# zdebruine/MMVAE

Hardware: AMD Instinct MI355X
Metric: cells/sec per MMVAE train step (higher is better)
Workload: dtype f32; 1 GPU; c2: 2-modality MMVAE train step, 20000 genes each, latent 128, K=1, batch 512/GPU, adversarial=False; global_batch=512, parallelism=dp1, exchange=none

## Files before the change

### include/mmvae_hip.h

```cpp
#ifndef MMVAE_HIP_H
#define MMVAE_HIP_H

#include <stddef.h>
#include <stdint.h>

#ifdef __cplusplus
extern "C" {
#endif

typedef void* mmvae_stream_t;

#define MMVAE_OK 0
#define MMVAE_ERR_ARG 1
#define MMVAE_ERR_LAUNCH 2
#define MMVAE_ERR_WORKSPACE 3

#define MMVAE_ABI_VERSION 16
int mmvae_abi_version(void);
const char* mmvae_build_arch(void);

#define MMVAE_GEMM_NT 0
#define MMVAE_GEMM_NN 1
#define MMVAE_GEMM_TN 2

// ... 197 lines not shown
typedef struct {
    const float* A;
    const float* B;
    float* C;
    const float* bias;
    int64_t lda, ldb, ldc;
    int32_t layout, M, N, K;
    float alpha;
    uint32_t flags;
    int32_t first_block;
    int32_t n_blocks;
} mmvae_gemm_job;
int mmvae_gemm_batch_job_ok(const mmvae_gemm_job* job);
int mmvae_gemm_batch_prepare(int n_jobs, mmvae_gemm_job* jobs, int* total_blocks);
int mmvae_gemm_batch_f32(int n_jobs, const mmvae_gemm_job* jobs_dev, int total_blocks, mmvae_stream_t stream);

int mmvae_csr_to_dense_f32(int B, int G, int64_t nnz, const int64_t* crow_indices, const int64_t* col_indices,
                           const float* values, float* out, int64_t ldo, mmvae_stream_t stream);
int mmvae_csr_to_dense_i32_f32(int B, int G, int64_t nnz, const int32_t* crow_indices, const int32_t* col_indices,
                               const float* values, float* out, int64_t ldo, mmvae_stream_t stream);

int mmvae_csr_gather_rows_i64(int B, int64_t n_src_rows, int64_t src_nnz, const int64_t* src_crow, const int64_t* src_col,
                              const float* src_val, const int64_t* rows, const int64_t* out_crow, int64_t out_nnz,
                              int64_t* out_col, float* out_val, mmvae_stream_t stream);
int mmvae_csr_gather_rows_i32(int B, int64_t n_src_rows, int64_t src_nnz, const int32_t* src_crow, const int32_t* src_col,
                              const float* src_val, const int64_t* rows, const int32_t* out_crow, int64_t out_nnz,
                              int32_t* out_col, float* out_val, mmvae_stream_t stream);
int mmvae_csr_gather_rows_dense_i64(int B, int G, int64_t n_src_rows, int64_t src_nnz, const int64_t* src_crow,
                                    const int64_t* src_col, const float* src_val, const int64_t* rows, float* out,
                                    int64_t ldo, mmvae_stream_t stream);
// ... 132 lines not shown
```

### mmvae_amd/_lib.py

```python
from __future__ import annotations

import ctypes as C
import os
from typing import Optional

_HERE = os.path.dirname(os.path.abspath(__file__))
LIB_PATH = os.path.join(_HERE, "csrc", "libmmvae_hip.so")
if os.environ.get("MMVAE_LIB"):
    LIB_PATH = os.environ["MMVAE_LIB"]

OK, ERR_ARG, ERR_LAUNCH, ERR_WORKSPACE = 0, 1, 2, 3
_ERR_NAMES = {1: "MMVAE_ERR_ARG", 2: "MMVAE_ERR_LAUNCH", 3: "MMVAE_ERR_WORKSPACE"}

GEMM_NT, GEMM_NN, GEMM_TN = 0, 1, 2
GEMM_RELU, GEMM_ACCUMULATE, GEMM_RAW_SLABS, GEMM_OPERAND_SLACK = 1, 2, 4, 8
GEMM_PRECISION_F32, GEMM_PRECISION_BF16X3 = 0, 1
ADAM_STATE_FLOATS = 8
ADAM_HYPER_FLOATS = 4
PREPARE_NORM, PREPARE_ADVANCE = 1, 2

_p = C.c_void_p
_i = C.c_int
_l = C.c_int64
_f = C.c_float
# ... 16 lines not shown


class Planes(C.Structure):
    _fields_ = [("p", _p), ("ld", _l), ("plane_stride", _l)]


class ReconArgs(C.Structure):
    _fields_ = [("rows", C.c_int32), ("x_rows", C.c_int32), ("G", C.c_int32), ("H", C.c_int32), ("flags", C.c_uint32),
                ("reserved", C.c_uint32), ("h", _p), ("W", _p), ("bias", _p), ("x", _p), ("ldh", _l), ("ldw", _l),
                ("ldx", _l), ("xhat", _p), ("dP", _p), ("se_part", _p), ("col_part", _p), ("ldxhat", _l), ("lddp", _l),
                ("h_planes", Planes), ("W_planes", Planes), ("dP_planes", Planes)]


class SplitJob(C.Structure):
    _fields_ = [("rows", C.c_int32), ("cols", C.c_int32), ("src", _p), ("ld_src", _l), ("planes", Planes)]


RECON_H_KPAD = 1


PROTOTYPES = {
    "mmvae_abi_version": (_i, []),
    "mmvae_build_arch": (C.c_char_p, []),
    "mmvae_gemm_set_precision": (_i, [_i]),
    "mmvae_gemm_set_workgroup_cap": (_i, [_i]),
    "mmvae_adam_set_workgroups": (_i, [_i]),
    "mmvae_adam_get_workgroups": (_i, []),
    "mmvae_gemm_set_x3w": (_i, [_i]),
    "mmvae_gemm_get_x3w": (_i, []),
    "mmvae_gemm_get_precision": (_i, []),
# ... 68 lines not shown
    "mmvae_csr_gather_rows_i64": (_i, [_i, _l, _l, _p, _p, _p, _p, _p, _l, _p, _p, _p]),
    "mmvae_csr_gather_rows_i32": (_i, [_i, _l, _l, _p, _p, _p, _p, _p, _l, _p, _p, _p]),
    "mmvae_csr_gather_rows_dense_i64": (_i, [_i, _i, _l, _l, _p, _p, _p, _p, _p, _l, _p]),
    "mmvae_csr_gather_rows_dense_i32": (_i, [_i, _i, _l, _l, _p, _p, _p, _p, _p, _l, _p]),
    "mmvae_csr_spmm_wt_i32_f32": (_i, [_i, _i, _i, _l, _p, _p, _p, _p, _l, _p, _p, _l, _p]),
    "mmvae_cond_linear_fwd": (_i, [_i, _i, _i, _p, _l, _p, _p, _p, _p, _p, _p, _l, _p]),
    "mmvae_cond_linear_bwd_dx": (_i, [_i, _i, _i, _p, _l, _p, _p, _p, _p, _p, _l, _i, _p]),
    "mmvae_cond_linear_bwd_dw": (_i, [_i, _p, _p, _p, _p, _i, _i, _p, _l, _p, _l, _p, _p, _p, _i, _p, _p, _p, _p, _p]),
    "mmvae_cond_linear_fwd_multi": (_i, [_i, _i, _i, _i, _p, _l, _l, _p, _p, _p, _p, _p, _l, _p, _l, _l, _p]),
    "mmvae_cond_linear_bwd_dx_multi": (_i, [_i, _i, _i, _i, _p, _l, _l, _p, _p, _p, _l, _p, _l, _i, _p]),
    "mmvae_cond_linear_bwd_dw_multi": (_i, [_i, _i, _p, _p, _p, _p, _l, _i, _i, _p, _l, _l, _p, _l, _l, _p, _p, _p, _i, _p,
                                            _p, _p, _p, _l, _p]),
    "mmvae_gemm_batch_job_ok": (_i, [_p]),
    "mmvae_gemm_batch_prepare": (_i, [_i, _p, C.POINTER(_i)]),
    "mmvae_gemm_batch_f32": (_i, [_i, _p, _i, _p]),
    "mmvae_adv_pass_plan": (_i, [_p, _i, C.POINTER(_i), C.POINTER(_z), C.POINTER(_l), C.POINTER(_i)]),
    "mmvae_adv_pass_f32": (_i, [_i, _p, _i, _i, _i, _i, _z, _p]),
    "mmvae_adv_dw_prepare": (_i, [_i, _p, C.POINTER(_i), C.POINTER(_i)]),
    "mmvae_adv_dw_f32": (_i, [_i, _p, _i, _i, _p, _p, _p, _i, _p, _i, _p]),
    "mmvae_adam_step_multi_hp": (_i, [_i, _p, _l, _p]),
    "mmvae_ell_from_dense_f32": (_i, [_i, _i, _p, _l, _i, _p, _p, _p, _p]),
    "mmvae_dw_sparse_ell_f32": (_i, [_i, _i, _i, _p, _l, _p, _p, _p, _i, _p, _l, _p]),
    "mmvae_col_pearson_workspace_bytes": (_z, [_i, _i]),
    "mmvae_col_pearson_f32": (_i, [_i, _i, _p, _l, _p, _l, _p, _p, _z, _p]),
}


class SumJob(C.Structure):
    _fields_ = [("src", C.c_void_p), ("dst", C.c_void_p), ("part_stride", C.c_int64), ("ld_src", C.c_int64),
                ("ld_dst", C.c_int64), ("n_parts", C.c_int32), ("rows", C.c_int32), ("cols", C.c_int32),
# ... 84 lines not shown
```

### mmvae_amd/csrc/gemm_dev.h

```cpp
#pragma once
#include "common.h"
#include <type_traits>

namespace mmvae_detail {
struct GemmArgs {
    const float* A;
    const float* B;
    float* C;
    const float* bias;
    int64_t lda, ldb, ldc;
    int M, N, K;
    int mt, nt;
    int ktiles;
    int ktiles_per_split;
    int64_t slab_stride;
    float alpha;
    unsigned flags;
    int aligned;
    int x3_vec;
    const float* x;
    float* xhat;
    float* dP;
    float* se_part;
    int64_t ldx, ldxhat, lddp;
    int x_rows;
    int se_tiles;
    int c_vec;
    int nwork;
    float* sq_part;
    float* col_part;
    const unsigned short* Ap;
    const unsigned short* Bp;
    int64_t ldap, ldbp, a_pstride, b_pstride;
    unsigned short* dPp;
    int64_t lddpp, dp_pstride;
};
bool x3w_planes_combo(int layout, bool a_pl, bool b_pl);
int launch_x3w_planes(int layout, int tile_id, bool a_pl, bool b_pl, int epi, const GemmArgs& g, int nwork, int slots,
                      hipStream_t s);

}

namespace {

#ifndef MMVAE_GEMM_BK0
#define MMVAE_GEMM_BK0 32
#endif
#ifndef MMVAE_X3_PERSISTENT
#define MMVAE_X3_PERSISTENT 0
#endif
#ifndef MMVAE_X3_STAMPS
#define MMVAE_X3_STAMPS 0
#endif
#ifndef MMVAE_SLAB_STORE_NT
#define MMVAE_SLAB_STORE_NT 0
#endif
#ifndef MMVAE_GEMM_PRELOAD
#define MMVAE_GEMM_PRELOAD 0
#endif

constexpr int NT = 256;

enum { FORM_KC = 0, FORM_RC = 1 };
enum { EPI_STD = 0, EPI_RECON = 1 };

template <int FORM, int R, int BK>
struct Tile {
    static constexpr int KC_LD = BK + 4;
    static constexpr int LDS_FLOATS = (FORM == FORM_KC) ? R * KC_LD : BK * R;
    static constexpr int NVEC = R * BK / 4;
    static constexpr int VECS = (NVEC + NT - 1) / NT;
    static constexpr bool EXACT = (NVEC % NT) == 0;
    static constexpr int C4 = (FORM == FORM_KC) ? BK / 4 : R / 4;
};

using mmvae_detail::GemmArgs;


template <int FORM, int R, int BK, bool VEC, int NV>
// ... 1571 lines not shown
```

### mmvae_amd/csrc/gemm_f32.hip

```cpp
#include "gemm_dev.h"

namespace {

template <int AFORM, int BFORM, int BM, int BN, int BK>
struct F32Lds {
    static constexpr int A_FLOATS = Tile<AFORM, BM, BK>::LDS_FLOATS, B_FLOATS = Tile<BFORM, BN, BK>::LDS_FLOATS;
    static constexpr int FLOATS = 2 * A_FLOATS + 2 * B_FLOATS;
};

template <int AFORM, int BFORM, int BM, int BN, int BK, int WGM, int WGN, bool VEC, int EPI>
__device__ __forceinline__ void gemm_f32_item(const GemmArgs& g, int L, float* lds) {
    static_assert(WGM * WGN == 4, "4 wavefronts per workgroup");
    constexpr int WTM = BM / WGM, WTN = BN / WGN;
    constexpr int TM = WTM / 32, TN = WTN / 32;
    static_assert(TM * 32 == WTM && TN * 32 == WTN && BK % 8 == 0, "tile shape");
    using TA = Tile<AFORM, BM, BK>;
    using TB = Tile<BFORM, BN, BK>;
    constexpr int A_FLOATS = TA::LDS_FLOATS, B_FLOATS = TB::LDS_FLOATS;
    constexpr int KK = BK / 8;
    float* As = lds;
    float* Bs = lds + 2 * A_FLOATS;

    const int tid = threadIdx.x;
    const int lane = tid & 63;
// ... 70 lines not shown
#pragma unroll
                    for (int i = 0; i < TM; ++i)
#pragma unroll
                        for (int n = 0; n < TN; ++n)
                            acc[i][n] = __builtin_amdgcn_mfma_f32_32x32x2f32(fa[i][j], fb[n][j], acc[i][n], 0, 0, 0);
            }
#endif
            if (more) {
                store_tile<AFORM, BM, BK>(As + (cur ^ 1) * A_FLOATS, ra, va, tid);
                store_tile<BFORM, BN, BK>(Bs + (cur ^ 1) * B_FLOATS, rb, vb, tid);
            }
            __syncthreads();
        }
    }

    gemm_epilogue<BM, BN, WGM, WGN, EPI>(acc, g, bm, bn, z, lds);
}

template <int AFORM, int BFORM, int BM, int BN, int BK, int WGM, int WGN, bool VEC, int EPI>
__global__ __launch_bounds__(NT) void gemm_f32_kernel(const GemmArgs g) {
    __shared__ __attribute__((aligned(16))) float lds[F32Lds<AFORM, BFORM, BM, BN, BK>::FLOATS];
    gemm_f32_item<AFORM, BFORM, BM, BN, BK, WGM, WGN, VEC, EPI>(g, xcd_remap(blockIdx.x, gridDim.x), lds);
}

__global__ __launch_bounds__(NT) void gemm_f32_batch_kernel(const mmvae_gemm_job* __restrict__ jobs, int n_jobs) {
    constexpr int LDS_FLOATS = F32Lds<FORM_KC, FORM_KC, 64, 64, 32>::FLOATS;
    static_assert(LDS_FLOATS >= F32Lds<FORM_KC, FORM_RC, 64, 64, 32>::FLOATS &&
                      LDS_FLOATS >= F32Lds<FORM_RC, FORM_RC, 64, 64, 32>::FLOATS, "LDS size");
    __shared__ __attribute__((aligned(16))) float lds[LDS_FLOATS];
    const int L = xcd_remap(blockIdx.x, gridDim.x);
    int j = 0;
// ... 1046 lines not shown
    *total_blocks = (int)first;
    return MMVAE_OK;
}

extern "C" int mmvae_gemm_batch_f32(int n_jobs, const mmvae_gemm_job* jobs_dev, int total_blocks,
                                    mmvae_stream_t stream) {
    if (n_jobs <= 0 || !jobs_dev || total_blocks <= 0) return MMVAE_ERR_ARG;
    if (x3s_enabled())
        MMVAE_LAUNCH(gemm_x3s_batch_kernel, dim3(total_blocks), dim3(NT), 0, (hipStream_t)stream, jobs_dev, n_jobs);
    else
        MMVAE_LAUNCH(gemm_f32_batch_kernel, dim3(total_blocks), dim3(NT), 0, (hipStream_t)stream, jobs_dev, n_jobs);
    MMVAE_LAUNCH_CHECK();
    return MMVAE_OK;
}

extern "C" int mmvae_recon_tiles(int G) {
    if (G <= 0) return 0;
    return ceil_div_i(G, g_precision == MMVAE_GEMM_PRECISION_BF16X3 ? 128 : 160);
}

#if MMVAE_X3_STAMPS
extern "C" int mmvae_debug_x3_stamps(long long* out32) {
    return hipMemcpyFromSymbol(out32, HIP_SYMBOL(g_x3_stamps), sizeof(long long) * 32) == hipSuccess ? 0 : 1;
}
extern "C" int mmvae_debug_x3_trace(long long* out, int n_blocks) {
    return hipMemcpyFromSymbol(out, HIP_SYMBOL(g_x3_trace), sizeof(long long) * 4 * n_blocks) == hipSuccess ? 0 : 1;
}
#endif

extern "C" int mmvae_gemm_set_precision(int mode) {
// ... 111 lines not shown
```

### mmvae_amd/engine.py

```python
from __future__ import annotations

import os
from dataclasses import dataclass
from typing import Dict, List, Optional

import torch

from . import _lib, dist as mdist, rng
from .constants import REGISTRY_KEYS as RK
from .engine_adv import PlanAdversaries
from .engine_common import ACC, NN, NT, RELU, SQ_FUSED_SLOTS, TN, _LayerRef, _PlaneBuf, _block_decline, _p
from .engine_cond import CondProgram
from .engine_emit import PlanEmit
from .engine_run import PlanRun
from .modules.base.components import Adversarial, FCBlock, _identity
from .optim import HipAdam

MAX_POINTER_PLANS = 8
SIDE_MAX_ROWS = 640
ADV_DW_CAP = 170


@dataclass(frozen=True)
class EngineSettings:
    conditionals: bool = True
    graphs: bool = True
    planes: bool = True
    side_dw: int = 125
    side_dw2: int = 185
    side_dw_dp: int = 125
    side_dw_any: bool = False
    prefetch_adv: int = 86
    cond_batched: bool = True
    prefetch: int = 128
    adv_fused: bool = True
    adv_aside: int = 2
    dp_overlap: Optional[bool] = None
    dp_shard: bool = True
    dp_kernels: str = "auto"
    dp_sim_world: int = 0
    dp_autotune_force: bool = False
    stamps: bool = False

    @staticmethod
    def from_env() -> "EngineSettings":
        e = os.environ.get
        ov = e("MMVAE_DP_OVERLAP", "")
        kernels = e("MMVAE_DP_KERNELS", "auto")
        if kernels not in ("auto", "dynamic", "persistent"):
            raise _lib.HipLibraryError(f"MMVAE_DP_KERNELS={kernels!r}: dynamic | persistent | auto")
        return EngineSettings(
            conditionals=e("MMVAE_ENGINE_CONDITIONALS", "1") != "0", graphs=e("MMVAE_NO_GRAPH", "0") == "0",
            planes=e("MMVAE_PLANES", "1") != "0", side_dw=int(e("MMVAE_SIDE_DW", "125")),
            side_dw2=int(e("MMVAE_SIDE_DW2", "185")), side_dw_dp=int(e("MMVAE_SIDE_DW_DP", "125")),
            side_dw_any=e("MMVAE_SIDE_DW_ANY", "0") != "0", prefetch=int(e("MMVAE_PREFETCH", "128")),
            cond_batched=e("MMVAE_COND_BATCHED", "1") != "0", prefetch_adv=int(e("MMVAE_PREFETCH_ADV", "86")),
            adv_fused=e("MMVAE_ADV_FUSED", "1") != "0",
            adv_aside=int(e("MMVAE_ADV_ASIDE", "2")),
            dp_overlap=None if ov == "" else ov != "0", dp_shard=e("MMVAE_DP_SHARD", "1") != "0", dp_kernels=kernels,
            dp_sim_world=int(e("MMVAE_DP_SIM_WORLD", "0")), dp_autotune_force=e("MMVAE_DP_AUTOTUNE_FORCE", "0") != "0",
            stamps=e("MMVAE_STAMPS", "0") == "1")


FORK_VALIDATED_RUNTIMES = ("7.0.",)


def concurrent_streams(device, n: int, pool: int = 12) -> list:
    main = torch.cuda.current_stream(device)
    spin = 400_000
    out = []
    for _ in range(pool):
        c = torch.cuda.Stream(device=device)
        torch.cuda.synchronize(device)
        t0, t1, m0, m1 = (torch.cuda.Event(enable_timing=True) for _ in range(4))
        ev = torch.cuda.Event()
        with torch.cuda.stream(c):
# ... 668 lines not shown
        self._gemm_jobs: List = []
        self._sum_jobs: List = []
        self._sum_keep: List = []
        self._job_tables: List = []
        self._ws_bytes = 0
        self._slab_floats = 0
        self._graphs: Optional[list] = None
        self._probe_next = None
        self.probe = None
        self.probe_meta: Dict[str, dict] = {}
        self._forked = False
        self._events: List = []
        self._runs = 0
        self.exp_norm_log = None
        self._x_split_jobs: List = []
        self._defer_next_dw = False
        self._deferred_dw = None
        self._fcws_bytes = 0
        self._defer_id = 0
        self.x_fp32_dw1 = False
        self.adv_grad_into: Dict[int, torch.Tensor] = {}
        self.n_adv = 0
        self._label_ring = None
        self._log_cache: Dict[tuple, list] = {}
        self.metrics = eng.buf("metrics", (256,))
        self.rng_state = rng.state(eng.device)
        cl = getattr(m.vae, "conditionals", None)
        self.cond = None
        if cl is not None and mode != "embed":
            if K != 1:
                raise _lib.HipLibraryError("engine: conditional layers with the K-sample extension are not supported")
            self.cond = CondProgram(self, cl, eid, train=(mode == "train"))
        self.layout = plan_layout(
            eng.settings, fork_ok=eng.fork_ok, side_stream=eng.side_stream is not None,
            side_stream2=eng.side_stream2 is not None, lane_stream=eng.lane_stream is not None, overlap=eng.overlap,
            world=eng.world, mode=mode, B=B, K=K, R=self.R, G=self.G, n_in_last=self.dec_layers[-1].n_in, iwae=self.iwae,
            has_adv=self.has_adv, has_cond=self.cond is not None,
            adv_reducer=any(o.reducer is not None for o in self.opt_adv))
        self._build()

    def _layer_refs(self, block: FCBlock) -> list:
        g = self.eng.grad_of
        return [_LayerRef(seq, g, block.config.return_hidden[i], block, i) for i, seq in enumerate(block.fc_layers)]

    def _build(self):
        self.eps = self.eng.buf("eps", (self.K, self.B, self.Z))
        self._mark("step begins (behind the noise fill)")
        self._plan_operand_planes()
        self._emit_encoder_forward()
        self._emit_heads()
        if self.mode == "embed":
            return self._finish_forward_only()
        if self.mode == "generate":
            self._emit_generate()
            return self._finish_forward_only()
        adv = self._emit_adversaries()
        loss_calls = self._emit_decoder_forward()
        if self.mode != "train":
# ... 121 lines not shown
                if adv_aside:
                    self._fork()
        return hidden, adv_calls, adv_aside, adv_lane

    def _adv_dp(self) -> bool:
        return self.eng.overlap or any(o.reducer is not None for o in self.opt_adv)

    def _emit_decoder_forward(self) -> list:
        eng, lib, L = self.eng, self.lib, self.layout
        B, K, R, Z, G, train = self.B, self.K, self.R, self.Z, self.G, self.mode == "train"
        cur, ld = self.z, Z
        if self.cond is not None:
            cur, ld = self.cond.emit_forward(self.z)
        for i, l in enumerate(self.dec_layers[:-1]):
            to_planes = self.hp is not None and K == 1 and i == len(self.dec_layers) - 2
            cur = self.fwd_layer(f"{self.eid}.dec{i}.K{K}", l, cur, ld, R, training=train,
                                 mask_stream=len(self.enc_layers) + i, planes_out=self.hp if to_planes else None,
                                 split_job=None if to_planes else self._next_x_split_job(l, R))
            ld = l.n_out
        for job in self._x_split_jobs:
            self._emit(lib.mmvae_split_planes_f32, *job)
        self._x_split_jobs = []
        last = self.dec_layers[-1]
        if not (last.relu and last.bn is None and last.ln is None and last.p == 0):
            raise _lib.HipLibraryError("engine: the last decoder layer must be Linear+ReLU (fused recon epilogue)")
        last.inp, last.ld_inp, last.rows = cur, ld, R
        T = lib.mmvae_recon_tiles(G)
        Gp = (G + 31) // 32 * 32
        if not (train and Gp != G and L.big and lib.mmvae_gemm_get_precision() == 1
                and (Gp - G) * last.n_in <= last.b.numel() + 32
                and last.b.data_ptr() == last.W.data_ptr() + 4 * last.W.numel()):
            Gp = G
        self.ldp = Gp
# ... 109 lines not shown
            self._mark("decoder dX done")
            if L.early:
                self._fork()
                self._branch(eng.side_stream, loss_calls + [c for c in [self._mark_call("decoder dW + loss words done (branch)")] if c])
        elif L.dp_dw and self._plan_gemm(TN, G, last.n_in, self.kpad(R)) == 1:
            S = self._emit_dec_dx()
            self._emit_dec_dw(last.inp, last.ld_inp, cap=L.dp_dw, exchange=True)
        else:
            self._emit_dec_dw(dw_inp, dw_ld, probe=L.big)
            S = self._emit_dec_dx(probe=L.big, planes=(None, self.wp) if self.pl_dec_w else None)
        rest = self.dec_layers[:-1]
        for j in range(len(rest) - 1, -1, -1):
            l = rest[j]
            rs = w_rows if j == len(rest) - 1 else None
            if j > 0:
                S = self.bwd_layer(l, None, S, need_dx="raw", row_scale=rs)
            else:
                self.bwd_layer(l, None, S, need_dx="full", row_scale=rs,
                               dx_out=self.dz_lat if self.cond is None else self.cond.d_out)
        if self.cond is not None:
            self.cond.emit_backward(self.dz_lat)
            if mdist.collectives_active():
                self._emit(lib.mmvae_grad_zero_flagged_jobs, self.cond.max_jobs, self.cond.jobs_ptr,
                           _p(self.cond.opt.arena.grad))
        if not rest:
            raise _lib.HipLibraryError("engine: decoder needs at least two layers")
        if adv_lane or adv_aside:
            self._mark("chain reaches the adversaries' join")
            if adv_lane:
                self._host_marker(("lane_join", eng.lane_stream))
            else:
# ... 160 lines not shown
```

### mmvae_amd/engine_emit.py

```python
from __future__ import annotations

import ctypes as C
from typing import Optional

import torch

from . import _lib, dist as mdist
from .engine_common import ACC, NN, NT, RAW, RELU, SLACK, SQ_FUSED_SLOTS, TN, _LayerRef, _NOPL, _PlaneBuf, _p, _planes_desc, _s
from .optim import HipAdam


class PlanEmit:
    def _emit(self, fn, *args, probe=None):
        lib_fn = fn

        def call():
            rc = lib_fn(*args, _s())
            if rc != 0:
                raise _lib.HipLibraryError(f"{lib_fn.__name__} failed with code {rc}")

        self._cur.append(self._probed(probe[0], probe[1], call) if probe else call)

    def _mark_call(self, name: str):
        if not self.eng.stamps:
# ... 201 lines not shown
        self._ws_bytes = max(self._ws_bytes, nbytes)
        self._gemm_launch(layout, M, N, K, alpha, A, lda, Bm, ldb, Cm, ldc, bias, flags, sk=sk, planes=planes, use_ws=True)

    def _edge(self, src, dst):
        ev = torch.cuda.Event()
        self._events.append(ev)

        def call():
            s = src if src is not None else torch.cuda.current_stream()
            d = dst if dst is not None else torch.cuda.current_stream()
            ev.record(s)
            d.wait_event(ev)

        self._cur.append(call)

    def _next_x_split_job(self, l: _LayerRef, rows: int):
        if not self._x_split_jobs:
            return None
        p_drop = l.p if self.mode == "train" else 0.0
        if l.ln is not None and l.bn is None:
            return None
        if l.bn is None and p_drop == 0 and self._plan_gemm(NT, rows, l.n_out, l.n_in) == 1:
            return None
        job = self._x_split_jobs.pop(0)
        return _lib.SplitJob(*job[:4], _lib.Planes(*job[4:]))

    def _fork(self, stream=None):
        side = stream if stream is not None else self.eng.side_stream
        self._edge(None, side)
        self._forked = True
        if side not in self._dirty:
            self._dirty.append(side)
# ... 34 lines not shown
    def _flush_sums(self):
        self._flush_gemms()
        if not self._sum_jobs:
            return
        arr = (_lib.SumJob * len(self._sum_jobs))(*self._sum_jobs)
        self._emit(self.lib.mmvae_sum_parts_batch, len(self._sum_jobs), self._upload_table(arr),
                   max(int(j.rows) * int(j.cols) for j in self._sum_jobs))
        self._sum_jobs = []

    def gemm_raw(self, layout, M, N, K, A, lda, Bm, ldb, planes=None) -> int:
        sk = self._plan_gemm(layout, M, N, K)
        self._slab_floats = max(self._slab_floats, sk * M * N)
        self._gemm_launch(layout, M, N, K, 1.0, A, lda, Bm, ldb, None, N, None, RAW, sk=sk, planes=planes)
        return sk

    def fwd_layer(self, tag: str, l: _LayerRef, cur: torch.Tensor, ld_cur: int, rows: int, training: bool = True,
                  mask_tag: Optional[str] = None, mask_stream: Optional[int] = None, planes_out: Optional[_PlaneBuf] = None,
                  split_job=None, slabs_from: Optional[torch.Tensor] = None):
        eng = self.eng
        l.inp, l.ld_inp, l.rows = cur, ld_cur, rows
        l.d = eng.buf(f"{tag}.d", (rows, l.n_out))
        l.z = eng.buf(f"{tag}.z", (rows, l.n_out)) if l.bn is not None else None
        l.mean = eng.buf(f"{tag}.mean", (l.n_out,)) if l.bn is not None else None
        l.invstd = eng.buf(f"{tag}.invstd", (l.n_out,)) if l.bn is not None else None
        l.mask = eng.buf(f"{mask_tag or tag}.mask", (rows, l.n_out), torch.uint8) if (l.p > 0 and training) else None
        if l.mask is not None:
            self._mask_layers.append((l, mask_stream if mask_stream is not None else len(self._mask_layers)))
        l.a = eng.buf(f"{tag}.a", (rows, l.n_out)) if (l.p > 0 and l.return_hidden and training) else None
        l.dz = eng.buf(f"{tag}.dz", (rows, l.n_out)) if training else None
        p_drop = l.p if training else 0.0
        self._fcws_bytes = max(self._fcws_bytes, self.lib.mmvae_fc_workspace_bytes(rows, l.n_out))
        sk = self._plan_gemm(NT, rows, l.n_out, l.n_in)
        l.y = l.ln_invstd = l.bn_out = l.dy = None
        if l.ln is not None:
            return self._fwd_layer_ln(tag, l, cur, ld_cur, rows, training, p_drop, sk, planes_out, split_job, slabs_from)
        if l.bn is None and p_drop == 0 and sk == 1:
            self.gemm(NT, rows, l.n_out, l.n_in, cur, ld_cur, l.W, l.n_in, l.d, l.n_out, bias=l.b,
                      flags=RELU if l.relu else 0)
            if planes_out is not None:
                self._emit(self.lib.mmvae_split_planes_f32, rows, l.n_out, _p(l.d), l.n_out, *planes_out.args())
            return l.d
        if slabs_from is not None:
            assert tuple(slabs_from.shape) == (sk, rows, l.n_out) and slabs_from.is_contiguous()
            S = sk
        else:
            S = self.gemm_raw(NT, rows, l.n_out, l.n_in, cur, ld_cur, l.W, l.n_in)
        self._emit_col_fwd(l, rows, S, slabs_from, training, l.relu, l.mask, p_drop, l.a, l.d, planes_out, split_job)
        return l.d

    def _emit_col_fwd(self, l: _LayerRef, rows: int, S: int, slabs_from, training: bool, relu: bool, mask, p_drop: float,
# ... 36 lines not shown

        def call():
            in_ptr = _p(src) if src is not None else (slabs_from.data_ptr() if slabs_from is not None else plan.slab.data_ptr())
            rc = plan.lib.mmvae_fc_rowtail_fwd(rows, l.n_out, in_ptr, l.n_out, S, _p(bias), l.ln, int(training), int(l.relu),
                                               _p(l.mask), p_drop, _p(l.y), _p(l.a), _p(l.d), l.n_out, _p(l.ln_invstd), _s())
            if rc != 0:
                raise _lib.HipLibraryError(f"mmvae_fc_rowtail_fwd failed with code {rc}")

        self._cur.append(call)
        if planes_out is not None:
            self._emit(self.lib.mmvae_split_planes_f32, rows, l.n_out, _p(l.d), l.n_out, *planes_out.args())
        return l.d

    def bwd_layer(self, l: _LayerRef, din, S_in: int, addend=None, need_dx: str = "raw", dx_out=None, dx_flags=0,
                  dx_alpha=1.0, dz_planes: Optional[_PlaneBuf] = None, inp_planes: Optional[_PlaneBuf] = None,
                  row_scale=None):
        rows = l.rows
        dw_planes = (dz_planes, inp_planes) if (dz_planes is not None and (inp_planes is not None or self.x_fp32_dw1)) else None
        dz_pl = _lib.Planes(*dz_planes.args()) if dw_planes is not None else None
        plan = self
        relu_src = l.a if l.a is not None else l.d
        has_bn = l.bn is not None

        own_ws = None
        if not has_bn and l.gb is not None:
            own_ws = self._bias_partials(rows, l.n_out, l.gb)
        after_ln = l.ln is not None
        if after_ln:
            din, S_in, addend, row_scale = self._bwd_layer_ln(l, din, S_in, addend, row_scale, own_ws)

        def call():
            din_ptr = _p(din) if din is not None else plan.slab.data_ptr()
            ws = own_ws if own_ws is not None else plan.fcws
            mask, relu = (None, False) if after_ln else (l.mask, l.relu)
            rc = plan.lib.mmvae_fc_epilogue_bwd(
                rows, l.n_out, din_ptr, l.n_out, S_in, None, _p(addend), _p(row_scale), _p(mask), l.p, int(relu),
                _p(relu_src) if relu else None, _p(l.z), _p(l.bn.weight) if has_bn else None, _p(l.mean),
                _p(l.invstd), int(has_bn), _p(l.dz), l.n_out, _p(l.gb) if own_ws is None else None,
                _p(l.ggamma) if has_bn else None, _p(l.gbeta) if has_bn else None, ws.data_ptr(), ws.numel() * 4,
                dz_pl, _s())
            if rc != 0:
                raise _lib.HipLibraryError(f"mmvae_fc_epilogue_bwd failed with code {rc}")

        if has_bn or not after_ln:
            self._cur.append(call)
        k_rows = rows if (self.K > 1 and l.inp is self.z and rows != self.R) else self.kpad(rows)
        if self._defer_next_dw:
            self._deferred_dw = ((TN, l.n_out, l.n_in, k_rows, l.dz, l.n_out, l.inp, l.ld_inp, l.gW, l.n_in), dw_planes)
            self._defer_next_dw = False
        else:
            big_first = l is self.enc_layers[0] and 2.0 * l.n_out * l.n_in * k_rows >= 5e9
            self._probe_next = "enc_l1_dw" if big_first else None
            self.gemm(TN, l.n_out, l.n_in, k_rows, l.dz, l.n_out, l.inp, l.ld_inp, l.gW, l.n_in, side=True, planes=dw_planes)
            self._probe_next = None
        if need_dx == "raw":
            return self.gemm_raw(NN, rows, l.n_in, l.n_out, l.dz, l.n_out, l.W, l.n_in)
        if need_dx == "full":
            if not self._gemm_group([(NN, rows, l.n_in, l.n_out, l.dz, l.n_out, l.W, l.n_in, dx_out, l.n_in, None,
                                      dx_flags, dx_alpha)]):
                self.gemm(NN, rows, l.n_in, l.n_out, l.dz, l.n_out, l.W, l.n_in, dx_out, l.n_in, flags=dx_flags,
                          alpha=dx_alpha)
        return 0

    def _bwd_layer_ln(self, l: _LayerRef, din, S_in: int, addend, row_scale, own_ws):
        plan, rows, has_bn = self, l.rows, l.bn is not None
        out = l.dy if has_bn else l.dz
        act = (l.a if l.a is not None else l.d) if l.relu else None
        y = l.y if l.y is not None else l.d

# ... 159 lines not shown
```

### mmvae_amd/ops.py

```python
from __future__ import annotations

import ctypes as C
from typing import Optional, Tuple

import torch

from . import _lib
from ._lib import GEMM_NT, GEMM_NN, GEMM_TN, GEMM_RELU, GEMM_ACCUMULATE, GEMM_RAW_SLABS

_workspaces: dict = {}


def _stream() -> int:
    return torch.cuda.current_stream().cuda_stream


def _chk(t: Optional[torch.Tensor], name: str, dtype=torch.float32) -> Optional[torch.Tensor]:
    if t is None:
        return None
    if not t.is_cuda:
        raise _lib.HipLibraryError(
            f"{name}: mmvae_amd HIP ops need a device tensor (got {t.device}); there is no CPU fallback. "
            "For CPU plumbing (BASELINE config C1) enable mmvae_amd.backend.cpu_plumbing()."
        )
# ... 179 lines not shown
        n = lib.mmvae_gemm_sq_partials(layout, M, N, Kk, 0)
        if n <= 0:
            raise ValueError("gemm_planes: this shape is planned as a split-K launch")
        partials = torch.empty(n, dtype=torch.float32, device=dev)
    rc = lib.mmvae_gemm_planes_f32(
        layout, M, N, Kk, 1.0,
        _ptr(a), a.stride(0) if a is not None else 0, a_planes.ptr() if a_planes else None,
        a_planes.ld if a_planes else 0, a_planes.plane_stride if a_planes else 0,
        _ptr(b), b.stride(0) if b is not None else 0, b_planes.ptr() if b_planes else None,
        b_planes.ld if b_planes else 0, b_planes.plane_stride if b_planes else 0,
        _ptr(out), ldc, None, flags, splitk, _ptr(ws), nbytes, _ptr(partials), n, _stream())
    _lib.check(rc, "mmvae_gemm_planes_f32")
    return (out, partials) if want_sq else out


def gemm_slabs(layout: int, a: torch.Tensor, b: torch.Tensor, splitk: int = 0) -> torch.Tensor:
    lib = _lib.load()
    _chk(a, "a"), _chk(b, "b")
    ar, ac, lda = _mat(a, "a")
    br, bc, ldb = _mat(b, "b")
    if layout == GEMM_NT:
        M, K, N = ar, ac, br
    elif layout == GEMM_NN:
        M, K, N = ar, ac, bc
    else:
        K, M, N = ar, ac, bc
    if splitk == 0:
        _, splitk = gemm_plan(layout, M, N, K)
    out = torch.empty((splitk, M, N), dtype=torch.float32, device=a.device)
    rc = lib.mmvae_gemm_f32(
# ... 650 lines not shown
```

Measured before the change: 580,300 cells/s.

## Fuse FC layer tail into single GEMM launch with epilogue bias/relu/planes/colsum

Adds a new GEMM kernel variant with an FC epilogue that applies bias, alpha, row scale and ReLU, masks by the activation, writes bf16x3 planes, and emits per-row-tile column partial sums. Decoder forward layers that were split-K or needed a separate plane split now run as one non-split launch, and the backward dx of a layer is fused with the ReLU-mask, bias-gradient tail of the layer below. This removes separate split-K reduction, epilogue and split kernels. In exchange it gives up split-K parallelism on those layers by forcing a fixed 64x64 tile.

```diff
diff --git a/include/mmvae_hip.h b/include/mmvae_hip.h
--- a/include/mmvae_hip.h
+++ b/include/mmvae_hip.h
@@ -235,6 +235,26 @@
 int mmvae_gemm_batch_job_ok(const mmvae_gemm_job* job);
 int mmvae_gemm_batch_prepare(int n_jobs, mmvae_gemm_job* jobs, int* total_blocks);
 int mmvae_gemm_batch_f32(int n_jobs, const mmvae_gemm_job* jobs_dev, int total_blocks, mmvae_stream_t stream);
+
+typedef struct mmvae_gemm_fc_args {
+    int32_t layout, M, N, K;
+    uint32_t flags;
+    int32_t splitk;
+    float alpha;
+    uint32_t reserved;
+    const float *A, *B, *bias;
+    int64_t lda, ldb;
+    float* C;
+    int64_t ldc;
+    mmvae_planes C_planes;
+    const float* act;
+    int64_t ldact;
+    const float* row_scale;
+    float* col_part;
+} mmvae_gemm_fc_args;
+int mmvae_gemm_fc_row_tiles(int M);
+size_t mmvae_sizeof_gemm_fc_args(void);
+int mmvae_gemm_fc_f32(const mmvae_gemm_fc_args* args, mmvae_stream_t stream);
 
 int mmvae_csr_to_dense_f32(int B, int G, int64_t nnz, const int64_t* crow_indices, const int64_t* col_indices,
                            const float* values, float* out, int64_t ldo, mmvae_stream_t stream);
diff --git a/mmvae_amd/_lib.py b/mmvae_amd/_lib.py
--- a/mmvae_amd/_lib.py
+++ b/mmvae_amd/_lib.py
@@ -54,6 +54,13 @@
 
 class SplitJob(C.Structure):
     _fields_ = [("rows", C.c_int32), ("cols", C.c_int32), ("src", _p), ("ld_src", _l), ("planes", Planes)]
+
+
+class GemmFcArgs(C.Structure):
+    _fields_ = [("layout", C.c_int32), ("M", C.c_int32), ("N", C.c_int32), ("K", C.c_int32), ("flags", C.c_uint32),
+                ("splitk", C.c_int32), ("alpha", _f), ("reserved", C.c_uint32), ("A", _p), ("B", _p), ("bias", _p),
+                ("lda", _l), ("ldb", _l), ("C", _p), ("ldc", _l), ("C_planes", Planes), ("act", _p), ("ldact", _l),
+                ("row_scale", _p), ("col_part", _p)]
 
 
 RECON_H_KPAD = 1
@@ -152,6 +159,9 @@
     "mmvae_gemm_batch_job_ok": (_i, [_p]),
     "mmvae_gemm_batch_prepare": (_i, [_i, _p, C.POINTER(_i)]),
     "mmvae_gemm_batch_f32": (_i, [_i, _p, _i, _p]),
+    "mmvae_gemm_fc_row_tiles": (_i, [_i]),
+    "mmvae_sizeof_gemm_fc_args": (_z, []),
+    "mmvae_gemm_fc_f32": (_i, [C.POINTER(GemmFcArgs), _p]),
     "mmvae_adv_pass_plan": (_i, [_p, _i, C.POINTER(_i), C.POINTER(_z), C.POINTER(_l), C.POINTER(_i)]),
     "mmvae_adv_pass_f32": (_i, [_i, _p, _i, _i, _i, _i, _z, _p]),
     "mmvae_adv_dw_prepare": (_i, [_i, _p, C.POINTER(_i), C.POINTER(_i)]),
diff --git a/mmvae_amd/csrc/gemm_dev.h b/mmvae_amd/csrc/gemm_dev.h
--- a/mmvae_amd/csrc/gemm_dev.h
+++ b/mmvae_amd/csrc/gemm_dev.h
@@ -34,6 +34,11 @@
     int64_t ldap, ldbp, a_pstride, b_pstride;
     unsigned short* dPp;
     int64_t lddpp, dp_pstride;
+    unsigned short* Cp;
+    int64_t ldcp, c_pstride;
+    const float* act;
+    int64_t ldact;
+    const float* row_scale;
 };
 bool x3w_planes_combo(int layout, bool a_pl, bool b_pl);
 int launch_x3w_planes(int layout, int tile_id, bool a_pl, bool b_pl, int epi, const GemmArgs& g, int nwork, int slots,
@@ -62,7 +67,7 @@
 constexpr int NT = 256;
 
 enum { FORM_KC = 0, FORM_RC = 1 };
-enum { EPI_STD = 0, EPI_RECON = 1 };
+enum { EPI_STD = 0, EPI_RECON = 1, EPI_FC = 2 };
 
 template <int FORM, int R, int BK>
 struct Tile {
diff --git a/mmvae_amd/csrc/gemm_f32.hip b/mmvae_amd/csrc/gemm_f32.hip
--- a/mmvae_amd/csrc/gemm_f32.hip
+++ b/mmvae_amd/csrc/gemm_f32.hip
@@ -7,6 +7,108 @@
     static constexpr int A_FLOATS = Tile<AFORM, BM, BK>::LDS_FLOATS, B_FLOATS = Tile<BFORM, BN, BK>::LDS_FLOATS;
     static constexpr int FLOATS = 2 * A_FLOATS + 2 * B_FLOATS;
 };
+
+template <int BM, int BN, int WGM, int WGN, int TM, int TN>
+__device__ __forceinline__ void fc_layer_epilogue(f32x16 (&acc)[TM][TN], const GemmArgs& g, int bm, int bn, float* lds) {
+    static_assert(TM == 1, "one row block per wave: the column sums of a wave are complete after one pass");
+    constexpr int WTM = BM / WGM, WTN = BN / WGN;
+    const int tid = threadIdx.x;
+    const int lane = tid & 63;
+    const int wave = tid >> 6;
+    const int wm = wave / WGN, wn = wave % WGN;
+    const int l31 = lane & 31, half = lane >> 5, q = lane & 3;
+    const bool odd = q & 1, hi = q & 2;
+    const bool relu = (g.flags & MMVAE_GEMM_RELU) != 0;
+    const int npad = (g.N + 7) & ~7;
+    float* colbuf = lds;
+#pragma unroll
+    for (int n = 0; n < TN; ++n) {
+        const int cloc = wn * WTN + n * 32 + (l31 & ~3);
+        const int col = bn * BN + cloc;
+        const int nv = g.N - col;
+        f32x4 bv = {0.f, 0.f, 0.f, 0.f};
+        if (g.bias && nv > 0) {
+            if (nv >= 4) {
+                bv = *reinterpret_cast<const f32x4*>(g.bias + col);
+            } else {
+                for (int j = 0; j < nv; ++j) bv[j] = g.bias[col + j];
+            }
+        }
+        f32x4 cs = {0.f, 0.f, 0.f, 0.f};
+#pragma unroll
+        for (int gq = 0; gq < 4; ++gq) {
+            const float a0 = acc[0][n][4 * gq], a1 = acc[0][n][4 * gq + 1], a2 = acc[0][n][4 * gq + 2],
+                        a3 = acc[0][n][4 * gq + 3];
+            const float r0 = quad_perm<1, 0, 3, 2>(odd ? a0 : a1), r1 = quad_perm<1, 0, 3, 2>(odd ? a2 : a3);
+            const float c0 = odd ? r0 : a0, c1 = odd ? a1 : r0, c2 = odd ? r1 : a2, c3 = odd ? a3 : r1;
+            const float t0 = quad_perm<2, 3, 0, 1>(hi ? c0 : c2), t1 = quad_perm<2, 3, 0, 1>(hi ? c1 : c3);
+            f32x4 v;
+            v[0] = hi ? t0 : c0;
+            v[1] = hi ? t1 : c1;
+            v[2] = hi ? c2 : t0;
+            v[3] = hi ? c3 : t1;
+            const int row = bm * BM + wm * WTM + 8 * gq + 4 * half + q;
+            if (row >= g.M || col >= npad) continue;
+            v = v * g.alpha + bv;
+            if (g.row_scale) v *= g.row_scale[row];
+            if (relu) {
+#pragma unroll
+                for (int j = 0; j < 4; ++j) v[j] = fmaxf(v[j], 0.f);
+            }
+            if (g.act && nv > 0) {
+                const float* ap = g.act + (int64_t)row * g.ldact + col;
+                f32x4 av = {0.f, 0.f, 0.f, 0.f};
+                if (nv >= 4) {
+                    av = *reinterpret_cast<const f32x4*>(ap);
+                } else {
+                    for (int j = 0; j < nv; ++j) av[j] = ap[j];
+                }
+#pragma unroll
+                for (int j = 0; j < 4; ++j) v[j] = (av[j] > 0.f) ? v[j] : 0.f;
+            }
+#pragma unroll
+            for (int j = 0; j < 4; ++j) v[j] = (j < nv) ? v[j] : 0.f;
+            float* cp = g.C + (int64_t)row * g.ldc + col;
+            if (nv >= 4) {
+                *reinterpret_cast<f32x4*>(cp) = v;
+            } else {
+                for (int j = 0; j < nv; ++j) cp[j] = v[j];
+            }
+            if (g.Cp) {
+                uint2 pk[3];
+                x3_pack4_lean(f32x2{v[0], v[1]}, f32x2{v[2], v[3]}, pk);
+                unsigned short* pp = g.Cp + (int64_t)row * g.ldcp + col;
+#pragma unroll
+                for (int pl = 0; pl < 3; ++pl) *reinterpret_cast<uint2*>(pp + pl * g.c_pstride) = pk[pl];
+            }
+            cs += v;
+        }
+        if (g.col_part) {
+#pragma unroll
+            for (int j = 0; j < 4; ++j) {
+                float s = cs[j];
+                s += __shfl_xor(s, 1, 64);
+                s += __shfl_xor(s, 2, 64);
+                s += __shfl_xor(s, 32, 64);
+                cs[j] = s;
+            }
+            if (q == 0 && half == 0) {
+#pragma unroll
+                for (int j = 0; j < 4; ++j) colbuf[wm * BN + cloc + j] = cs[j];
+            }
+        }
+    }
+    if (g.col_part) {
+        __syncthreads();
+        const int col = bn * BN + tid;
+        if (tid < BN && col < g.N) {
+            float s = colbuf[tid];
+#pragma unroll
+            for (int w = 1; w < WGM; ++w) s += colbuf[w * BN + tid];
+            g.col_part[(int64_t)bm * g.N + col] = s;
+        }
+    }
+}
 
 template <int AFORM, int BFORM, int BM, int BN, int BK, int WGM, int WGN, bool VEC, int EPI>
 __device__ __forceinline__ void gemm_f32_item(const GemmArgs& g, int L, float* lds) {
@@ -108,7 +210,10 @@
         }
     }
 
-    gemm_epilogue<BM, BN, WGM, WGN, EPI>(acc, g, bm, bn, z, lds);
+    if constexpr (EPI == EPI_FC)
+        fc_layer_epilogue<BM, BN, WGM, WGN>(acc, g, bm, bn, lds);
+    else
+        gemm_epilogue<BM, BN, WGM, WGN, EPI>(acc, g, bm, bn, z, lds);
 }
 
 template <int AFORM, int BFORM, int BM, int BN, int BK, int WGM, int WGN, bool VEC, int EPI>
@@ -1185,6 +1290,67 @@
     return MMVAE_OK;
 }
 
+extern "C" int mmvae_gemm_fc_row_tiles(int M) { return M > 0 ? ceil_div_i(M, 64) : 0; }
+extern "C" size_t mmvae_sizeof_gemm_fc_args(void) { return sizeof(mmvae_gemm_fc_args); }
+
+template <int AFORM, int BFORM>
+static int launch_gemm_fc(const GemmArgs& g, hipStream_t s) {
+    const int nblocks = g.mt * g.nt;
+    if (g.aligned == 2)
+        MMVAE_LAUNCH((gemm_f32_kernel<AFORM, BFORM, 64, 64, 32, 2, 2, true, EPI_FC>), dim3(nblocks), dim3(NT), 0, s, g);
+    else
+        MMVAE_LAUNCH((gemm_f32_kernel<AFORM, BFORM, 64, 64, 32, 2, 2, false, EPI_FC>), dim3(nblocks), dim3(NT), 0, s, g);
+    MMVAE_LAUNCH_CHECK();
+    return MMVAE_OK;
+}
+
+extern "C" int mmvae_gemm_fc_f32(const mmvae_gemm_fc_args* args, mmvae_stream_t stream) {
+    if (!args) return MMVAE_ERR_ARG;
+    const mmvae_gemm_fc_args& a = *args;
+    if (a.layout != MMVAE_GEMM_NT && a.layout != MMVAE_GEMM_NN) return MMVAE_ERR_ARG;
+    if (a.M <= 0 || a.N <= 0 || a.K <= 0 || !a.A || !a.B || !a.C) return MMVAE_ERR_ARG;
+    if (a.splitk != 1 || a.reserved != 0 || (a.flags & ~MMVAE_GEMM_RELU)) return MMVAE_ERR_ARG;
+    if (a.lda < a.K || a.ldb < (a.layout == MMVAE_GEMM_NT ? a.K : a.N) || a.ldc < a.N) return MMVAE_ERR_ARG;
+    if ((int64_t)ceil_div_i(a.M, 64) * ceil_div_i(a.N, 64) > (1 << 30)) return MMVAE_ERR_ARG;
+    if (a.act && a.ldact < a.N) return MMVAE_ERR_ARG;
+    const mmvae_planes& cp = a.C_planes;
+    if (cp.p && (!aligned16(cp.p) || cp.ld % 8 != 0 || cp.ld < ((int64_t)a.N + 7) / 8 * 8 || cp.plane_stride % 8 != 0 ||
+                 cp.plane_stride < (int64_t)a.M * cp.ld || 3 * cp.plane_stride * 2 >= (int64_t)0xFFFFFFFF))
+        return MMVAE_ERR_ARG;
+    GemmArgs g = {};
+    g.A = a.A;
+    g.B = a.B;
+    g.C = a.C;
+    g.bias = a.bias;
+    g.lda = a.lda;
+    g.ldb = a.ldb;
+    g.ldc = a.ldc;
+    g.M = a.M;
+    g.N = a.N;
+    g.K = a.K;
+    g.mt = ceil_div_i(a.M, 64);
+    g.nt = ceil_div_i(a.N, 64);
+    g.ktiles = ceil_div_i(a.K, 32);
+    g.ktiles_per_split = g.ktiles;
+    g.alpha = a.alpha;
+    g.flags = a.flags;
+    g.x_rows = 1;
+    g.c_vec = 1;
+    int aligned = aligned16(a.A) && aligned16(a.B) && (a.lda % 4 == 0) && (a.ldb % 4 == 0);
+    if (aligned && a.M % 4 == 0 && a.N % 4 == 0 && a.K % 4 == 0) aligned = 2;
+    g.aligned = aligned;
+    g.Cp = reinterpret_cast<unsigned short*>(cp.p);
+    g.ldcp = cp.ld;
+    g.c_pstride = cp.plane_stride;
+    g.act = a.act;
+    g.ldact = a.ldact;
+    g.row_scale = a.row_scale;
+    g.col_part = a.col_part;
+    hipStream_t s = (hipStream_t)stream;
+    if (a.layout == MMVAE_GEMM_NT) return launch_gemm_fc<FORM_KC, FORM_KC>(g, s);
+    return launch_gemm_fc<FORM_KC, FORM_RC>(g, s);
+}
+
 extern "C" int mmvae_recon_tiles(int G) {
     if (G <= 0) return 0;
     return ceil_div_i(G, g_precision == MMVAE_GEMM_PRECISION_BF16X3 ? 128 : 160);
diff --git a/mmvae_amd/engine.py b/mmvae_amd/engine.py
--- a/mmvae_amd/engine.py
+++ b/mmvae_amd/engine.py
@@ -19,6 +19,7 @@
 MAX_POINTER_PLANS = 8
 SIDE_MAX_ROWS = 640
 ADV_DW_CAP = 170
+FC_ONE_LAUNCH_DEFAULT = "f1,f2"
 
 
 @dataclass(frozen=True)
@@ -41,6 +42,7 @@
     dp_sim_world: int = 0
     dp_autotune_force: bool = False
     stamps: bool = False
+    fc_one_launch: str = FC_ONE_LAUNCH_DEFAULT
 
     @staticmethod
     def from_env() -> "EngineSettings":
@@ -59,7 +61,7 @@
             adv_aside=int(e("MMVAE_ADV_ASIDE", "2")),
             dp_overlap=None if ov == "" else ov != "0", dp_shard=e("MMVAE_DP_SHARD", "1") != "0", dp_kernels=kernels,
             dp_sim_world=int(e("MMVAE_DP_SIM_WORLD", "0")), dp_autotune_force=e("MMVAE_DP_AUTOTUNE_FORCE", "0") != "0",
-            stamps=e("MMVAE_STAMPS", "0") == "1")
+            stamps=e("MMVAE_STAMPS", "0") == "1", fc_one_launch=e("MMVAE_FC_ONE_LAUNCH", FC_ONE_LAUNCH_DEFAULT))
 
 
 FORK_VALIDATED_RUNTIMES = ("7.0.",)
@@ -758,6 +760,7 @@
         self._runs = 0
         self.exp_norm_log = None
         self._x_split_jobs: List = []
+        self.fc_one_launch: List[str] = []
         self._defer_next_dw = False
         self._deferred_dw = None
         self._fcws_bytes = 0
@@ -786,6 +789,17 @@
     def _layer_refs(self, block: FCBlock) -> list:
         g = self.eng.grad_of
         return [_LayerRef(seq, g, block.config.return_hidden[i], block, i) for i, seq in enumerate(block.fc_layers)]
+
+    def _one_launch(self, kind: str, i: int) -> bool:
+        eng, v = self.eng, self.eng.settings.fc_one_launch
+        if v in ("", "0") or self.mode != "train" or eng.world > 1 or eng.overlap or self.K != 1 or self.R > SIDE_MAX_ROWS:
+            return False
+        if self.has_adv:
+            return False
+        return v in ("1", "all") or f"{kind}{i}" in v.split(",")
+
+    def program_calls(self) -> int:
+        return sum(len(seg) for seg in self.segments if isinstance(seg, list))
 
     def _build(self):
         self.eps = self.eng.buf("eps", (self.K, self.B, self.Z))
@@ -937,9 +951,10 @@
             cur, ld = self.cond.emit_forward(self.z)
         for i, l in enumerate(self.dec_layers[:-1]):
             to_planes = self.hp is not None and K == 1 and i == len(self.dec_layers) - 2
+            one = self._one_launch("f", i) and (to_planes or not self._x_split_jobs)
             cur = self.fwd_layer(f"{self.eid}.dec{i}.K{K}", l, cur, ld, R, training=train,
                                  mask_stream=len(self.enc_layers) + i, planes_out=self.hp if to_planes else None,
-                                 split_job=None if to_planes else self._next_x_split_job(l, R))
+                                 split_job=None if to_planes else self._next_x_split_job(l, R, one), one_launch=one)
             ld = l.n_out
         for job in self._x_split_jobs:
             self._emit(lib.mmvae_split_planes_f32, *job)
@@ -1079,7 +1094,8 @@
             l = rest[j]
             rs = w_rows if j == len(rest) - 1 else None
             if j > 0:
-                S = self.bwd_layer(l, None, S, need_dx="raw", row_scale=rs)
+                S = self.bwd_layer(l, None, S, need_dx="raw", row_scale=rs,
+                                   below=rest[j - 1] if self._one_launch("b", j - 1) else None)
             else:
                 self.bwd_layer(l, None, S, need_dx="full", row_scale=rs,
                                dx_out=self.dz_lat if self.cond is None else self.cond.d_out)
diff --git a/mmvae_amd/engine_emit.py b/mmvae_amd/engine_emit.py
--- a/mmvae_amd/engine_emit.py
+++ b/mmvae_amd/engine_emit.py
@@ -5,9 +5,12 @@
 
 import torch
 
-from . import _lib, dist as mdist
+from . import _lib, dist as mdist, ops
 from .engine_common import ACC, NN, NT, RAW, RELU, SLACK, SQ_FUSED_SLOTS, TN, _LayerRef, _NOPL, _PlaneBuf, _p, _planes_desc, _s
 from .optim import HipAdam
+
+
+TAIL_DONE = -1
 
 
 class PlanEmit:
@@ -239,8 +242,10 @@
 
         self._cur.append(call)
 
-    def _next_x_split_job(self, l: _LayerRef, rows: int):
+    def _next_x_split_job(self, l: _LayerRef, rows: int, one_launch: bool = False):
         if not self._x_split_jobs:
+            return None
+        if one_launch and ops.fc_tail_in_gemm(l.bn is not None, l.ln is not None, l.p if self.mode == "train" else 0.0):
             return None
         p_drop = l.p if self.mode == "train" else 0.0
         if l.ln is not None and l.bn is None:
@@ -305,9 +310,39 @@
         self._gemm_launch(layout, M, N, K, 1.0, A, lda, Bm, ldb, None, N, None, RAW, sk=sk, planes=planes)
         return sk
 
+    def _emit_gemm_fc(self, layout, M, N, K, A, lda, Bm, ldb, Cm, bias=None, relu=False, planes_out=None, act=None,
+                      row_scale=None, col_part=None):
+        args = _lib.GemmFcArgs(layout=layout, M=M, N=N, K=K, flags=RELU if relu else 0, splitk=1, alpha=1.0, A=_p(A),
+                               B=_p(Bm), bias=_p(bias), lda=lda, ldb=ldb, C=_p(Cm), ldc=N,
+                               C_planes=_lib.Planes(*planes_out.args()) if planes_out is not None else _lib.Planes(),
+                               act=_p(act), ldact=N, row_scale=_p(row_scale), col_part=_p(col_part))
+        self._sum_keep.append((A, Bm, Cm, bias, act, row_scale, col_part))
+        lib = self.lib
+
+        def call():
+            rc = lib.mmvae_gemm_fc_f32(C.byref(args), _s())
+            if rc != 0:
+                raise _lib.HipLibraryError(f"mmvae_gemm_fc_f32 failed with code {rc} (layout {layout}, {M}x{N}x{K})")
+
+        self._cur.append(call)
+
+    def _emit_dx_into_tail(self, l: _LayerRef, below: _LayerRef):
+        rows, N = l.rows, l.n_in
+        mt = self.lib.mmvae_gemm_fc_row_tiles(rows)
+        parts = self.eng.buf(f"biasparts.{self._next_defer_id()}", (mt, N))
+        self._defer_sum(parts, mt, N, 1, N, N, below.gb, N)
+        self._emit_gemm_fc(NN, rows, N, l.n_out, l.dz, l.n_out, l.W, l.n_in, below.dz,
+                           act=below.d if below.relu else None, col_part=parts)
+        self.fc_one_launch.append(f"backward tail of a {below.n_in}->{below.n_out} layer")
+
+    @staticmethod
+    def _tail_fits_gemm(below: _LayerRef) -> bool:
+        return (ops.fc_tail_in_gemm(below.bn is not None, below.ln is not None, below.p) and below.mask is None
+                and below.a is None and below.gb is not None and below.dz is not None)
+
     def fwd_layer(self, tag: str, l: _LayerRef, cur: torch.Tensor, ld_cur: int, rows: int, training: bool = True,
                   mask_tag: Optional[str] = None, mask_stream: Optional[int] = None, planes_out: Optional[_PlaneBuf] = None,
-                  split_job=None, slabs_from: Optional[torch.Tensor] = None):
+                  split_job=None, slabs_from: Optional[torch.Tensor] = None, one_launch: bool = False):
         eng = self.eng
         l.inp, l.ld_inp, l.rows = cur, ld_cur, rows
         l.d = eng.buf(f"{tag}.d", (rows, l.n_out))
@@ -325,6 +360,13 @@
         l.y = l.ln_invstd = l.bn_out = l.dy = None
         if l.ln is not None:
             return self._fwd_layer_ln(tag, l, cur, ld_cur, rows, training, p_drop, sk, planes_out, split_job, slabs_from)
+        if (one_launch and slabs_from is None and ops.fc_tail_in_gemm(False, False, p_drop) and l.bn is None
+                and (sk > 1 or planes_out is not None)):
+            assert split_job is None
+            self._emit_gemm_fc(NT, rows, l.n_out, l.n_in, cur, ld_cur, l.W, l.n_in, l.d, bias=l.b, relu=l.relu,
+                               planes_out=planes_out)
+            self.fc_one_launch.append(f"forward {tag}")
+            return l.d
         if l.bn is None and p_drop == 0 and sk == 1:
             self.gemm(NT, rows, l.n_out, l.n_in, cur, ld_cur, l.W, l.n_in, l.d, l.n_out, bias=l.b,
                       flags=RELU if l.relu else 0)
@@ -391,7 +433,7 @@
 
     def bwd_layer(self, l: _LayerRef, din, S_in: int, addend=None, need_dx: str = "raw", dx_out=None, dx_flags=0,
                   dx_alpha=1.0, dz_planes: Optional[_PlaneBuf] = None, inp_planes: Optional[_PlaneBuf] = None,
-                  row_scale=None):
+                  row_scale=None, below: Optional[_LayerRef] = None):
         rows = l.rows
         dw_planes = (dz_planes, inp_planes) if (dz_planes is not None and (inp_planes is not None or self.x_fp32_dw1)) else None
         dz_pl = _lib.Planes(*dz_planes.args()) if dw_planes is not None else None
@@ -399,8 +441,11 @@
         relu_src = l.a if l.a is not None else l.d
         has_bn = l.bn is not None
 
+        tail_done = S_in == TAIL_DONE
+        if tail_done:
+            assert din is None and addend is None and row_scale is None and dz_planes is None and self._tail_fits_gemm(l)
         own_ws = None
-        if not has_bn and l.gb is not None:
+        if not has_bn and l.gb is not None and not tail_done:
             own_ws = self._bias_partials(rows, l.n_out, l.gb)
         after_ln = l.ln is not None
         if after_ln:
@@ -419,7 +464,7 @@
             if rc != 0:
                 raise _lib.HipLibraryError(f"mmvae_fc_epilogue_bwd failed with code {rc}")
 
-        if has_bn or not after_ln:
+        if (has_bn or not after_ln) and not tail_done:
             self._cur.append(call)
         k_rows = rows if (self.K > 1 and l.inp is self.z and rows != self.R) else self.kpad(rows)
         if self._defer_next_dw:
@@ -430,6 +475,9 @@
             self._probe_next = "enc_l1_dw" if big_first else None
             self.gemm(TN, l.n_out, l.n_in, k_rows, l.dz, l.n_out, l.inp, l.ld_inp, l.gW, l.n_in, side=True, planes=dw_planes)
             self._probe_next = None
+        if need_dx == "raw" and below is not None and self._tail_fits_gemm(below):
+            self._emit_dx_into_tail(l, below)
+            return TAIL_DONE
         if need_dx == "raw":
             return self.gemm_raw(NN, rows, l.n_in, l.n_out, l.dz, l.n_out, l.W, l.n_in)
         if need_dx == "full":
diff --git a/mmvae_amd/ops.py b/mmvae_amd/ops.py
--- a/mmvae_amd/ops.py
+++ b/mmvae_amd/ops.py
@@ -217,6 +217,48 @@
     return (out, partials) if want_sq else out
 
 
+def fc_tail_in_gemm(has_bn: bool, has_ln: bool, p_drop: float) -> bool:
+    return not has_bn and not has_ln and p_drop == 0
+
+
+def gemm_fc(layout: int, a: torch.Tensor, b: torch.Tensor, *, out: Optional[torch.Tensor] = None,
+            bias: Optional[torch.Tensor] = None, alpha: float = 1.0, relu: bool = False, planes: Optional[Planes] = None,
+            act: Optional[torch.Tensor] = None, row_scale: Optional[torch.Tensor] = None, col_parts: bool = False,
+            splitk: int = 1):
+    lib = _lib.load()
+    _chk(a, "a"), _chk(b, "b"), _chk(bias, "bias"), _chk(act, "act"), _chk(row_scale, "row_scale")
+    M, K, lda = _mat(a, "a")
+    br, bc, ldb = _mat(b, "b")
+    N = br if layout == GEMM_NT else bc
+    if (bc if layout == GEMM_NT else br) != K:
+        raise ValueError(f"gemm_fc: a {tuple(a.shape)} vs b {tuple(b.shape)}")
+    if out is None:
+        out = torch.empty((M, N), dtype=torch.float32, device=a.device)
+    _chk(out, "out")
+    if tuple(out.shape) != (M, N) or (planes is not None and (planes.rows, planes.cols) != (M, N)):
+        raise ValueError("gemm_fc: output shape mismatch")
+    if (bias is not None and bias.numel() != N) or (row_scale is not None and row_scale.numel() != M):
+        raise ValueError("gemm_fc: bias [N] / row_scale [M]")
+    ldact = 0
+    if act is not None:
+        if tuple(act.shape) != (M, N):
+            raise ValueError("gemm_fc: act must be [M, N]")
+        ldact = _mat(act, "act")[2]
+    part = None
+    if isinstance(col_parts, torch.Tensor):
+        part = _chk(col_parts, "col_parts")
+        if tuple(part.shape) != (lib.mmvae_gemm_fc_row_tiles(M), N) or not part.is_contiguous():
+            raise ValueError("gemm_fc: col_parts must be contiguous [mmvae_gemm_fc_row_tiles(M), N]")
+    elif col_parts:
+        part = torch.empty((lib.mmvae_gemm_fc_row_tiles(M), N), dtype=torch.float32, device=a.device)
+    args = _lib.GemmFcArgs(layout=layout, M=M, N=N, K=K, flags=GEMM_RELU if relu else 0, splitk=splitk, alpha=alpha,
+                           A=_ptr(a), B=_ptr(b), bias=_ptr(bias), lda=lda, ldb=ldb, C=_ptr(out), ldc=_mat(out, "out")[2],
+                           C_planes=_c_planes(planes), act=_ptr(act), ldact=ldact, row_scale=_ptr(row_scale),
+                           col_part=_ptr(part))
+    _lib.check(lib.mmvae_gemm_fc_f32(C.byref(args), _stream()), "mmvae_gemm_fc_f32")
+    return out, part
+
+
 def gemm_slabs(layout: int, a: torch.Tensor, b: torch.Tensor, splitk: int = 0) -> torch.Tensor:
     lib = _lib.load()
     _chk(a, "a"), _chk(b, "b")
```

Result: no change. 581,000 cells/s, median of 5 (+0.1%).
